# jagannatharjun/AntiZ

Hardware: AMD Instinct MI355X
Metric: input MB/s precompressed (1 GB synthetic, 100k streams) at 1/2/4/8 MI355X (higher is better)
Workload: dtype u8

## Files before the change

antiz_amd/csrc/atz_device.h:

```cpp
#pragma once
#include <stdint.h>

#ifndef ATZ_INF_CLOCKS
#define ATZ_INF_CLOCKS 0
#endif

namespace atz {

struct InfJob {
  uint64_t in_off;
  uint64_t in_len;
  uint64_t out_off;
  uint64_t out_cap;
};
static constexpr uint64_t NO_OUT = ~0ull;
static constexpr uint64_t ARENA_OUT = ~1ull;
static constexpr uint64_t ARENA_NONE = ~0ull;

enum : uint32_t { INF_END = 0, INF_ERROR = 1, INF_NEED = 2, INF_RETRY = 3 };

static constexpr uint32_t INF_HINT_NOSHORT = 1u << 31;
static constexpr uint32_t INF_HINT_MLEV_SHIFT = 27;

struct InfRes {
// ... 81 lines not shown
  TR_FULL = 0,
  TR_SHORTCUT = 1,
  TR_SIZEDIFF = 2,
  TR_CANT_BEAT = 3,
  TR_OVERFLOW = 4,
  TR_NEED_R = 5,
  TR_SKIPPED = 6,
};

struct SweepOpts {
  uint64_t recomp_tresh, sizediff_tresh, shortcut_len, mismatch_tol;
};

__device__ __forceinline__ uint32_t wave_incl_scan(uint32_t v) {
  int x = (int)v;
  x += __builtin_amdgcn_update_dpp(0, x, 0x111, 0xf, 0xf, false);
  x += __builtin_amdgcn_update_dpp(0, x, 0x112, 0xf, 0xf, false);
  x += __builtin_amdgcn_update_dpp(0, x, 0x114, 0xf, 0xf, false);
  x += __builtin_amdgcn_update_dpp(0, x, 0x118, 0xf, 0xf, false);
  x += __builtin_amdgcn_update_dpp(0, x, 0x142, 0xa, 0xf, false);
  x += __builtin_amdgcn_update_dpp(0, x, 0x143, 0xc, 0xf, false);
  return (uint32_t)x;
}

}
```

antiz_amd/csrc/k_deflate.hip:

```cpp
#include <hip/hip_runtime.h>
#include "atz_device.h"

#define LDS __attribute__((address_space(3)))
#define CONSTANT __attribute__((address_space(4)))
#define GLOBAL __attribute__((address_space(1)))

#ifndef ATZ_VISITED_CHECK
#define ATZ_VISITED_CHECK 1
#endif
#ifndef ATZ_VISITED_MAX
#define ATZ_VISITED_MAX 8
#endif
#ifndef ATZ_NOSLIDE_PATH
#define ATZ_NOSLIDE_PATH 1
#endif
#ifndef ATZ_STEP_SPLIT
#define ATZ_STEP_SPLIT 0
#endif
#ifndef ATZ_STEP_CLOCKS
#define ATZ_STEP_CLOCKS 0
#endif
#if ATZ_STEP_CLOCKS
#define STEP_CLOCK() clock64()
#else
// ... 712 lines not shown
  uint32_t heap[HEAPN + 1];
  uint16_t bl_count[16];
  uint32_t blc32[16];
};

struct TreeScratch {
  uint16_t anc[2][HEAPN];
  uint8_t dep[2][HEAPN];
  uint16_t freq[NLC];
};

struct BitOut {
  GLOBAL uint8_t* out;
  uint64_t cap;
  uint64_t pos;
  uint64_t bb;
  uint32_t bc;
  uint32_t raw;
  const GLOBAL uint8_t* orig;
  uint64_t clen;
  uint64_t shortcut;
  uint64_t eq_all;
  uint64_t eq_sc;
  int overflow;
  uint64_t cyc_tree, cyc_emit, blocks;
  uint64_t cyc_heap, cyc_scan, cyc_send;
};

static constexpr uint32_t STAGE_WORDS = 196;
struct BlockFreq {
  uint32_t lfreq2[(NLC + 1) / 2];
  uint32_t dfreq2[NDC / 2];
};
struct TreeCodes {
  uint16_t lcode[NLC]; uint8_t llen[NLC + 2];
  uint16_t dcode[NDC]; uint8_t dlen[NDC + 2];
  uint16_t bcode[NBLC]; uint8_t blen[NBLC + 2];
  uint32_t bfreq[NBLC];
  TreeWork w;
};
struct TrialShared {
  BitOut b;
  BlockFreq f;
  TreeCodes k;
  uint64_t stop_at;
  uint32_t stop_j, pad_;
};

template <uint32_t INS>
struct TrialSharedFast {
  static constexpr uint32_t INS_BITS = INS;
  TrialShared t;
  uint64_t ring[512];
  uint32_t ins[INS / 32];
  uint32_t holes[HOLE_SLOTS];
};

static constexpr uint32_t RING_SLOW = 512;
struct TrialSharedSlow {
  TrialShared t;
  uint64_t ring[RING_SLOW];
};
static_assert(sizeof(TreeScratch) <= RING_SLOW * sizeof(uint64_t), "tree scratch overlays the ring");
static_assert(offsetof(BitOut, cyc_scan) == offsetof(BitOut, cyc_heap) + 8, "block_trees' cyc[0], cyc[1]");
static_assert(STAGE_WORDS * 4 <= RING_SLOW * sizeof(uint64_t), "emission staging overlays the ring");

#ifndef ATZ_MW_F
#define ATZ_MW_F 3
#endif
static constexpr int MW_F = ATZ_MW_F;
struct MWSlot {
  BlockFreq f;
  int64_t block_start;
  uint64_t p, S;
  uint32_t last_lit, sbase, last, seq;
};
struct MWFlusher {
  TreeCodes k;
  TreeScratch sc;
  uint64_t cyc_tree, cyc_emit;
  uint64_t cyc_heap, cyc_scan;
};
static_assert(offsetof(MWFlusher, cyc_scan) == offsetof(MWFlusher, cyc_heap) + 8, "block_trees' cyc[0], cyc[1]");
struct MWCtl {
  uint32_t next_emit;
  uint32_t stop;
  uint32_t parse_done, nblocks;
  uint32_t state, hazard;
// ... 24 lines not shown
__device__ __forceinline__ uint32_t ld_acq(const LDS uint32_t& x) {
  return uni(__hip_atomic_load(&x, __ATOMIC_ACQUIRE, __HIP_MEMORY_SCOPE_WORKGROUP));
}
__device__ __forceinline__ void st_rel(LDS uint32_t& x, uint32_t v, int lane) {
  if (lane == 0) __hip_atomic_store(&x, v, __ATOMIC_RELEASE, __HIP_MEMORY_SCOPE_WORKGROUP);
}

struct SweepArgs {
  const uint8_t* file;
  const uint8_t* infl;
  const uint32_t* chains;
  const uint2* R;
  const StreamDev* streams;
  const Trial* trials;
  TrialRes* res;
  uint32_t* stopj;
  uint8_t* out;
  uint32_t* syms;
  const uint32_t* adler;
  SweepOpts o;
  uint32_t ntrials;
};

__device__ inline uint64_t wsum64(uint64_t v) {
  for (int d = 32; d >= 1; d >>= 1) {
    uint32_t lo = __shfl_xor((uint32_t)v, d, 64), hi = __shfl_xor((uint32_t)(v >> 32), d, 64);
    v += ((uint64_t)hi << 32) | lo;
  }
  return v;
}

__device__ inline void emit_bytes_from_stage(LDS BitOut& b, const LDS uint32_t* stage, uint32_t nb, int lane) {
  uint32_t eqa = 0, eqs = 0;
  nb = uni(nb);
  const uint64_t pos = uni(b.pos), cap = uni(b.cap), clen = uni(b.clen), sc = uni(b.shortcut);
  GLOBAL uint8_t* const out = (GLOBAL uint8_t*)(uintptr_t)uni((uint64_t)(uintptr_t)b.out);
  const GLOBAL uint8_t* const orig = (const GLOBAL uint8_t*)(uintptr_t)uni((uint64_t)(uintptr_t)b.orig);
  for (uint32_t w = (uint32_t)lane; 4 * w < nb; w += 64) {
    const uint32_t word = stage[w];
#pragma unroll
    for (uint32_t j = 0; j < 4; j++) {
      const uint32_t k = 4 * w + j;
      const uint8_t x = (uint8_t)(word >> (8 * j));
      const uint64_t at = pos + k;
      if (k < nb && at < cap) out[at] = x;
      if (k < nb && at < clen) {
        const uint32_t e = orig[at] == x ? 1u : 0u;
        eqa += e;
        if (at < sc) eqs += e;
      }
    }
  }
  b.eq_all += wsum64(eqa);
  b.eq_sc += wsum64(eqs);
  if (pos + nb > cap) b.overflow = 1;
  b.pos = pos + nb;
}

__device__ inline void put_bits(LDS BitOut& b, LDS uint32_t* stage, uint32_t v, uint32_t n, int lane) {
  const uint32_t bc = uni(b.bc) + n;
  const uint64_t bb = uni(b.bb) | ((uint64_t)uni(v) << uni(b.bc));
  if (bc >= 32) {
    if (lane == 0) stage[0] = (uint32_t)bb;
    emit_bytes_from_stage(b, stage, 4, lane);
    b.bb = bb >> 32;
    b.bc = bc - 32;
  } else {
    b.bb = bb;
    b.bc = bc;
  }
}
__device__ inline void flush_bits_bytes(LDS BitOut& b, LDS uint32_t* stage, int lane) {
  const uint32_t bc = uni(b.bc), nb = bc >> 3;
  if (!nb) return;
  const uint64_t bb = uni(b.bb);
  if (lane == 0) { stage[0] = (uint32_t)bb; stage[1] = (uint32_t)(bb >> 32); }
  emit_bytes_from_stage(b, stage, nb, lane);
  b.bb = nb >= 8 ? 0 : (bb >> (8 * nb));
  b.bc = bc - 8 * nb;
}
__device__ inline void windup(LDS BitOut& b, LDS uint32_t* stage, int lane) {
  flush_bits_bytes(b, stage, lane);
  if (uni(b.bc)) {
    if (lane == 0) stage[0] = (uint32_t)b.bb;
    emit_bytes_from_stage(b, stage, 1, lane);
    b.bb = 0; b.bc = 0;
  }
}

__device__ __forceinline__ uint32_t tkey(uint32_t f, uint32_t d, uint32_t n) { return (f << 15) | (d << 10) | n; }

__device__ __forceinline__ void pq_down(LDS uint32_t* heap, int heap_len, int k, int lane) {
  const uint32_t v = uni(heap[k]);
  const uint32_t vk = v >> 10;
  const int t_l = 31 - __builtin_clz((uint32_t)lane + 2u);
  const int off_l = lane + 2 - (1 << t_l);
  for (;;) {
    if (2 * k > heap_len) break;
    const int idx = (k << t_l) + off_l;
    const uint32_t g = (t_l <= 5 && idx <= heap_len) ? heap[idx] : 0xffffffffu;
    int p = k;
    bool stop = false;
    int lj = 0;
#pragma unroll
    for (int t = 1; t <= 5; t++) {
      const uint32_t hl = (uint32_t)__builtin_amdgcn_readlane((int)g, lj);
      const uint32_t hr = (uint32_t)__builtin_amdgcn_readlane((int)g, lj + 1);
      const uint32_t c = (hr >> 10) <= (hl >> 10) ? 1u : 0u;
      const uint32_t hj = c ? hr : hl;
// ... 156 lines not shown
  if (overflow) {
    auto bl = [&](int b) -> uint32_t { return (uint32_t)__builtin_amdgcn_readlane((int)blc, b); };
    auto blset = [&](int b, uint32_t v) { blc = lane == b ? v : blc; };
    do {
      int bits = max_length - 1;
      while (bl(bits) == 0) bits--;
      blset(bits, bl(bits) - 1);
      blset(bits + 1, bl(bits + 1) + 2);
      blset(max_length, bl(max_length) - 1);
      overflow -= 2;
    } while (overflow > 0);
    int h = HEAPN;
    for (int bits = max_length; bits != 0; bits--) {
      uint32_t cnt = bl(bits);
      while (cnt != 0) {
        const uint32_t m = uni(heap[--h]);
        if ((int)m > max_code) continue;
        if (lane == 0) lenv[m] = (uint8_t)bits;
        cnt--;
      }
    }
  }
  if (lane < 16) w.bl_count[lane] = (uint16_t)blc;
  uint64_t o = 0, st = 0;
  for (int n = lane; n < elems && n <= max_code; n += 64) {
    const uint32_t f = sc.freq[n];
    if (f) {
      const uint32_t l = lenv[n];
      const uint32_t xb = (xbits && n >= xbase) ? xbits[n - xbase] : 0u;
      o += (uint64_t)f * (l + xb);
      if (stlen) st += (uint64_t)f * (stlen[n] + xb);
    }
  }
  opt_len += wsum64(o);
  if (stlen) static_len += wsum64(st);
  return TreeRes{max_code, opt_len, static_len};
}

__device__ __noinline__ void gen_codes(const LDS TreeWork& w, int max_code, LDS uint16_t* codes, LDS uint8_t* lens,
                                       int lane) {
  max_code = (int)uni((uint32_t)max_code);
  const bool lb = lane >= 1 && lane <= 15;
  const uint32_t bc = lb ? (uint32_t)w.bl_count[lane] : 0u;
  const uint32_t wv = bc << ((15 - lane) & 15);
  uint32_t nc = lb ? (wave_incl_scan(wv) - wv) >> (15 - lane) : 0u;
  const uint64_t lt = lane ? (~0ull >> (64 - lane)) : 0ull;
  const uint64_t present = __ballot(bc != 0);
  for (int g = 0; g <= max_code; g += 64) {
    const int n = g + lane;
    const uint32_t l = n <= max_code ? lens[n] : 0u;
    uint32_t mine = 0;
    for (uint64_t pm = present; pm; pm &= pm - 1) {
      const int b = __ffsll((unsigned long long)pm) - 1;
      const uint64_t m = __ballot(l == (uint32_t)b);
      if (!m) continue;
      const uint32_t base = (uint32_t)__builtin_amdgcn_readlane((int)nc, b);
      if (l == (uint32_t)b) mine = base + (uint32_t)__popcll(m & lt);
      if (lane == b) nc += (uint32_t)__popcll(m);
// ... 1 lines not shown
    if (n <= max_code && l) codes[n] = (uint16_t)(__builtin_bitreverse32(mine) >> (32 - l));
  }
}

__device__ __forceinline__ uint32_t len_code(uint32_t len) {
  if (len < 8) return len;
  if (len == 255) return 28;
  const uint32_t lg = 31u - (uint32_t)__clz(len);
  return 4u * (lg - 1u) + ((len >> (lg - 2u)) & 3u);
}
__device__ __forceinline__ uint32_t dist_code(uint32_t d) {
  if (d < 4) return d;
  const uint32_t lg = 31u - (uint32_t)__clz(d);
  return 2u * lg + ((d >> (lg - 1u)) & 1u);
}
__device__ __forceinline__ uint32_t lcode_extra(uint32_t c) { return (c < 8 || c == 28) ? 0u : (c - 4) >> 2; }
__device__ __forceinline__ uint32_t lcode_base(uint32_t c) {
  return c < 8 ? c : c == 28 ? 255u : ((4 + (c & 3)) << lcode_extra(c));
}
__device__ __forceinline__ uint32_t dcode_extra(uint32_t d) { return d < 2 ? 0u : (d >> 1) - 1; }
__device__ __forceinline__ uint32_t dcode_base(uint32_t d) { return d < 2 ? d : ((2 + (d & 1)) << dcode_extra(d)); }


__device__ inline uint32_t early_exit(const LDS BitOut& b, const SweepOpts& o, uint64_t best_ident, bool full_needed) {
  if (uni((uint32_t)b.overflow)) return TR_OVERFLOW;
  if (full_needed) return ~0u;
  const uint64_t pos = uni(b.pos), clen = uni(b.clen), sc = uni(b.shortcut);
  if (sc) {
    uint64_t seen = pos < sc ? pos : sc;
    uint64_t mism = seen - uni(b.eq_sc);
    uint64_t thr = o.shortcut_len - o.recomp_tresh;
    if (thr > sc || mism > sc - thr) return TR_SHORTCUT;
  }
  if (pos > clen + o.sizediff_tresh) return TR_SIZEDIFF;
  uint64_t seen = pos < clen ? pos : clen;
  if (clen - (seen - uni(b.eq_all)) <= best_ident) return TR_CANT_BEAT;
  return ~0u;
}

static constexpr uint32_t SYM_PER_LANE = 2;
template <typename C16, typename C8>
__device__ __forceinline__ void sym_bits(uint32_t sy, bool valid, bool end, C16 lc, C8 ll, C16 dc, C8 dl,
                                         uint64_t& v, uint32_t& nb) {
  v = 0; nb = 0;
  if (valid) {
    uint32_t dist = sy >> 8;
    const uint32_t c = sy & 0xff;
    if (dist == 0) {
      v = lc[c]; nb = ll[c];
    } else {
      const uint32_t code = len_code(c);
      v = lc[code + 257]; nb = ll[code + 257];
      const uint32_t xe = lcode_extra(code);
      if (xe) { v |= (uint64_t)(c - lcode_base(code)) << nb; nb += xe; }
      dist--;
      const uint32_t dcd = dist_code(dist);
      v |= (uint64_t)dc[dcd] << nb; nb += dl[dcd];
      const uint32_t xd = dcode_extra(dcd);
      if (xd) { v |= (uint64_t)(dist - dcode_base(dcd)) << nb; nb += xd; }
    }
  } else if (end) {
    v = lc[256]; nb = ll[256];
  }
// ... 67 lines not shown
            if (first) { v64 = cv; nb = cl; }
            v64 |= (uint64_t)s.bcode[16] << nb; nb += s.blen[16];
            v64 |= (uint64_t)(cnt - (first ? 1 : 0) - 3) << nb; nb += 2;
          } else if (cnt <= 10) {
            v64 = s.bcode[17]; nb = s.blen[17];
            v64 |= (uint64_t)(cnt - 3) << nb; nb += 3;
          } else {
            v64 = s.bcode[18]; nb = s.blen[18];
            v64 |= (uint64_t)(cnt - 11) << nb; nb += 7;
          }
        }
      }
    }
    if (send) {
      const uint32_t incl = wave_incl_scan(nb);
      stage_or(stage, off + incl - nb, v64, nb);
      off += (uint32_t)__builtin_amdgcn_readlane((int)incl, 63);
    }
  }
  return off;
}

template <typename C16, typename C8>
__device__ bool compress_block(LDS BitOut& b, LDS uint32_t* stage, const GLOBAL uint32_t* syms, uint32_t nsym,
                               C16 lc, C8 ll, C16 dc, C8 dl, const SweepOpts& o, uint64_t best_ident,
                               bool full_needed, int lane) {
  __builtin_amdgcn_fence(__ATOMIC_ACQ_REL, "workgroup");
  for (uint32_t base = 0; base <= nsym; base += 64 * SYM_PER_LANE) {
    const uint32_t k0 = base + SYM_PER_LANE * (uint32_t)lane;
    const uint64_t sp = *(const GLOBAL uint64_t*)(syms + k0);
    uint64_t v0, v1;
    uint32_t n0, n1;
    sym_bits((uint32_t)sp, k0 < nsym, k0 == nsym, lc, ll, dc, dl, v0, n0);
    sym_bits((uint32_t)(sp >> 32), k0 + 1 < nsym, k0 + 1 == nsym, lc, ll, dc, dl, v1, n1);
    const uint32_t nb = n0 + n1;
    const uint32_t incl = wave_incl_scan(nb);
    const uint32_t total = (uint32_t)__builtin_amdgcn_readlane((int)incl, 63);
    if (total == 0) break;
    for (int i = lane; i < (int)STAGE_WORDS; i += 64) stage[i] = 0;
    const uint32_t bc = uni(b.bc);
    if (lane == 0) { stage[0] = (uint32_t)b.bb; stage[1] = (uint32_t)(b.bb >> 32); }
    const uint32_t off = bc + incl - nb;
    stage_or(stage, off, v0, n0);
    stage_or(stage, off + n0, v1, n1);
    const uint32_t all = bc + total;
    const uint32_t full = all >> 3;
    emit_bytes_from_stage(b, stage, full, lane);
    const uint32_t rem = all & 7;
    const uint32_t lastw = stage[full >> 2];
    b.bb = rem ? ((lastw >> (8 * (full & 3))) & 0xff) & ((1u << rem) - 1) : 0;
    b.bc = rem;
    if (!full_needed && early_exit(b, o, best_ident, false) != ~0u) return true;
  }
  return false;
}

struct Lz {
  uint32_t level, kind, wsize, maxdist, lbs, good, lazy, nice, chain;
  uint32_t n;
  uint32_t p;
  uint32_t lookahead;
  uint32_t S;
  uint32_t block_start;
  uint32_t match_start, prev_match;
  uint32_t match_length, prev_length;
  int match_available;
  uint32_t last_lit;
  uint32_t nsym;
};

// ... 84 lines not shown
                                            int max_blindex, int lane) {
  syms = uni_ptr(syms);
  in = uni_ptr(in);
  block_start = (int64_t)uni((uint64_t)block_start);
  p = uni(p);
  S = uni(S);
  last_lit = uni(last_lit);
  lbs = uni(lbs);
  last = (int)uni((uint32_t)last);
  opt.recomp_tresh = uni(opt.recomp_tresh);
  opt.sizediff_tresh = uni(opt.sizediff_tresh);
  opt.shortcut_len = uni(opt.shortcut_len);
  opt.mismatch_tol = uni(opt.mismatch_tol);
  best_ident = uni(best_ident);
  full_needed = uni((uint32_t)full_needed) != 0;
  opt_lenb = uni(opt_lenb);
  static_lenb = uni(static_lenb);
  lmax = (int)uni((uint32_t)lmax);
  dmax = (int)uni((uint32_t)dmax);
  max_blindex = (int)uni((uint32_t)max_blindex);
  uint32_t hazard = 0;
  const bool bufok = block_start >= (int64_t)S;
  const uint64_t stored_len = (uint64_t)((int64_t)p - block_start);
  const uint64_t blk_start_bytes = b.pos;
  b.blocks++;
  if (stored_len + 4 <= opt_lenb && bufok) {
    put_bits(b, stage, (uint32_t)last, 3, lane);
    windup(b, stage, lane);
    uint32_t len = (uint32_t)stored_len;
    put_bits(b, stage, (len & 0xffff) | ((~len & 0xffff) << 16), 32, lane);
    const GLOBAL uint8_t* src = in + block_start;
    for (uint64_t o = 0; o < stored_len; o += 256) {
      uint32_t nb = stored_len - o < 256 ? (uint32_t)(stored_len - o) : 256u;
      for (uint32_t k = lane; k < 64; k += 64) {
        uint32_t wv = 0;
        for (int q = 0; q < 4; q++) {
          uint32_t at = 4 * k + q;
          if (at < nb) wv |= (uint32_t)src[o + at] << (8 * q);
        }
        stage[k] = wv;
      }
      emit_bytes_from_stage(b, stage, nb, lane);
      if (!full_needed && early_exit(b, opt, best_ident, false) != ~0u) break;
    }
  } else if (static_lenb == opt_lenb) {
    const uint32_t bc0 = uni(b.bc);
    b.bb = uni(b.bb) | ((uint64_t)((1u << 1) + (uint32_t)last) << bc0);
    b.bc = bc0 + 3;
    compress_block(b, stage, syms, last_lit, (const CONSTANT uint16_t*)c_t.st_lcode, (const CONSTANT uint8_t*)c_t.st_llen,
                   (const CONSTANT uint16_t*)c_t.st_dcode, (const CONSTANT uint8_t*)c_t.st_dlen, opt, best_ident,
                   full_needed, lane);
  } else {
    int lcodes = lmax + 1, dcodes = dmax + 1, blcodes = max_blindex + 1;
    const uint64_t cs0 = STEP_CLOCK();
    for (int i = lane; i < (int)STAGE_WORDS; i += 64) stage[i] = 0;
    const uint32_t bc0 = uni(b.bc);
    const uint64_t bb0 = uni(b.bb);
    if (lane == 0) { stage[0] = (uint32_t)bb0; stage[1] = (uint32_t)(bb0 >> 32); }
    uint32_t off = bc0;
    if (lane == 0)
      stage_or(stage, off, (uint64_t)((2u << 1) + (uint32_t)last) | ((uint64_t)(lcodes - 257) << 3) |
                               ((uint64_t)(dcodes - 1) << 8) | ((uint64_t)(blcodes - 4) << 13), 17);
    off += 17;
    if (lane < blcodes) stage_or(stage, off + 3u * (uint32_t)lane, s.blen[bl_order((uint32_t)lane)], 3);
    off += 3u * (uint32_t)blcodes;
    off = rle_tree(s, stage, s.llen, lcodes - 1, true, off, lane);
    off = rle_tree(s, stage, s.dlen, dcodes - 1, true, off, lane);
    {
      const uint32_t full = off >> 3;
      emit_bytes_from_stage(b, stage, full, lane);
      const uint32_t rem = off & 7;
      const uint32_t lastw = stage[full >> 2];
      b.bb = rem ? ((lastw >> (8 * (full & 3))) & 0xff) & ((1u << rem) - 1) : 0;
      b.bc = rem;
    }
    b.cyc_send += STEP_CLOCK() - cs0;
    compress_block(b, stage, syms, last_lit, (const LDS uint16_t*)s.lcode, (const LDS uint8_t*)s.llen,
                   (const LDS uint16_t*)s.dcode, (const LDS uint8_t*)s.dlen, opt, best_ident, full_needed, lane);
  }
  if (b.pos - blk_start_bytes > (uint64_t)lbs + 2ull * last_lit && last_lit) hazard = 1;
  if (last) windup(b, stage, lane);
  return hazard;
}

__device__ __forceinline__ void init_block(LDS BlockFreq& f, int lane) {
  for (int i = lane; i < (NLC + 1) / 2; i += 64) f.lfreq2[i] = 0;
  for (int i = lane; i < NDC / 2; i += 64) f.dfreq2[i] = 0;
  if (lane == 0) f.lfreq2[128] = 1;
}

__device__ __forceinline__ uint32_t flush_block(LDS TrialShared& s, LDS TreeScratch& sc, LDS BitOut& b, const GLOBAL uint32_t* syms,
                                                const GLOBAL uint8_t* in, int64_t block_start, uint64_t p, uint64_t S,
                                                uint32_t last_lit, uint32_t level, uint32_t lbs, int last, const SweepOpts& opt,
                                                uint64_t best_ident, bool full_needed, int lane) {
  const uint64_t c0 = clock64();
  const BlockPlan pl = block_trees(s.f, s.k, sc, &b.cyc_heap, level, (uint64_t)((int64_t)p - block_start), lane);
  const uint64_t c1 = clock64();
  b.cyc_tree += c1 - c0;
  const uint32_t hz = block_emit(s.k, (LDS uint32_t*)&sc, b, syms, in, block_start, p, S, last_lit, lbs, last, opt, best_ident,
                                 full_needed, pl.opt_lenb, pl.static_lenb, pl.lmax, pl.dmax, pl.max_blindex, lane);
  init_block(s.f, lane);
  b.cyc_emit += clock64() - c1;
  return hz;
}
// ... 93 lines not shown
    }
    if (!have) break;
    const int64_t bs = (int64_t)uni((uint64_t)sl.block_start);
    const uint64_t p = uni(sl.p), S = uni(sl.S);
    const uint32_t last_lit = uni(sl.last_lit), sbase = uni(sl.sbase);
    const int last = (int)uni(sl.last);
    const uint64_t c0 = clock64();
    const BlockPlan pl = block_trees(sl.f, me.k, me.sc, &me.cyc_heap, level, (uint64_t)((int64_t)p - bs), lane);
    st_rel(sl.seq, 0u, lane);
    const uint64_t c1 = clock64();
    bool turn = false;
    for (;;) {
      if (ld_acq(ctl.stop)) break;
      if (ld_acq(ctl.next_emit) == k) { turn = true; break; }
      __builtin_amdgcn_s_sleep(1);
    }
    if (!turn) break;
    const uint64_t c2 = clock64();
    const uint32_t hz = uni(block_emit(me.k, stage, b, syms + sbase, in, bs, p, S, last_lit, lbs, last, A.o, tr.best_ident,
                                       full_needed, pl.opt_lenb, pl.static_lenb, pl.lmax, pl.dmax, pl.max_blindex, lane));
    if (hz && lane == 0) __hip_atomic_fetch_or(&ctl.hazard, 1u, __ATOMIC_RELAXED, __HIP_MEMORY_SCOPE_WORKGROUP);
    uint32_t st = ~0u;
    if (last) {
      if (!uni(b.raw)) {
        const uint32_t ad = A.adler[tr.stream];
        const uint32_t be = ((ad >> 24) & 0xff) | ((ad >> 8) & 0xff00) | ((ad << 8) & 0xff0000) | (ad << 24);
        put_bits(b, stage, be, 32, lane);
      }
      flush_bits_bytes(b, stage, lane);
      if (uni((uint32_t)b.overflow)) st = TR_OVERFLOW;
      else if (full_needed) st = TR_FULL;
      else {
        const uint64_t thr = A.o.shortcut_len - A.o.recomp_tresh;
        const uint64_t L = uni(b.pos), clen = uni(b.clen);
        const int64_t dd = (int64_t)(L - clen);
        const uint64_t ad2 = (uint64_t)(dd < 0 ? -dd : dd);
        if (uni(b.shortcut) && uni(b.eq_sc) < thr) st = TR_SHORTCUT;
        else if (ad2 > A.o.sizediff_tresh) st = TR_SIZEDIFF;
        else st = TR_FULL;
      }
    } else {
      st = uni(early_exit(b, A.o, tr.best_ident, full_needed));
    }
    if (lane == 0) { me.cyc_tree += c1 - c0; me.cyc_emit += clock64() - c2; }
    if (last) spec_stop(s, A, tr.best_ident, st, uni(b.eq_all), uni(b.clen), lane);
    if (st != ~0u) {
      if (lane == 0) ctl.state = st;
      st_rel(ctl.stop, 1u, lane);
    }
    st_rel(ctl.next_emit, k + 1, lane);
    if (st != ~0u) break;
  }
}

static constexpr uint32_t TR_DECIDED = 0xfffffffeu;

template <int KIND, typename SH, int STRAT = 0>
struct TrialRun {
  static constexpr bool MW = HasMW<SH>::value;
  static constexpr bool TAB = KIND == 1 || KIND == 2;
  const SweepArgs& A;
  SH& shm;
  const int lane, wave;
  LDS TrialShared& s;
  LDS uint32_t* const stg;
  LDS BitOut& b;
  const uint32_t t;
  const Trial tr;
  const StreamDev sd;
  const uint8_t* const in;
  const uint32_t npad;
  const uint32_t* const sidx;
  const uint32_t* const bpos;
  const bool full_needed;
  const uint64_t lt;
  Lz z;
  bool saving = false, replay = false, rec = false;
  GLOBAL uint32_t* syms = nullptr;
  GLOBAL uint64_t* rtab = nullptr;
  uint32_t sbase = 0;
  uint32_t saved_flags = 0;
  uint32_t run_len = 0, run_imp = 0;
  uint64_t cstart = 0;
  uint32_t rtstart = 0;
  uint32_t hazard = 0;
  uint32_t state = ~0u;
  uint64_t fallbacks = 0, cyc_fb = 0;
  uint64_t csec[4] = {0, 0, 0, 0};
  uint32_t nblk = 0;
  LDS uint64_t* ring = nullptr;
  const GLOBAL uint64_t* Rt = nullptr;
  uint32_t n = 0, wsz = 0, maxd = 0, xlim = 0;
  bool noslide = false;
  uint32_t hi = 0;
  uint64_t pf = 0;
  LDS uint32_t* holes = nullptr;
  LDS uint32_t* ins = nullptr;

  __device__ __forceinline__ TrialRun(const SweepArgs& A_, SH& shm_, int lane_)
      : A(A_), shm(shm_), lane(lane_), wave(MW ? (int)(threadIdx.x >> 6) : 0), s(*(LDS TrialShared*)&shm_.t),
        stg((LDS uint32_t*)shm_.ring), b(s.b), t(blockIdx.x), tr(A_.trials[t]), sd(A_.streams[tr.stream]),
        in(A_.infl + sd.infl_off), npad((uint32_t)((sd.infl_len + 63) & ~63ull)),
        sidx(!TAB ? nullptr : A_.chains + tr.chain_off), bpos(!TAB ? nullptr : sidx + npad),
        full_needed(tr.mode & TM_FULL), lt(lane_ ? (~0ull >> (64 - lane_)) : 0ull) {
    z.level = tr.clevel; z.kind = KIND;
    z.wsize = 1u << tr.window; z.maxdist = z.wsize - LOOKMIN; z.lbs = 1u << (tr.memlevel + 6);
    z.good = c_cfg[z.level][0]; z.lazy = c_cfg[z.level][1]; z.nice = c_cfg[z.level][2]; z.chain = c_cfg[z.level][3];
    z.n = sd.infl_len; z.p = 0; z.lookahead = 0; z.S = 0; z.block_start = 0;
    z.match_start = 0; z.prev_match = 0; z.match_length = 2; z.prev_length = 2; z.match_available = 0;
    z.last_lit = 0; z.nsym = 0;
    if (wave == 0) {
      b.out = (GLOBAL uint8_t*)(A.out + tr.out_off); b.cap = tr.out_cap; b.pos = 0; b.bb = 0; b.bc = 0;
      b.raw = tr.mode & TM_RAW;
      b.orig = (const GLOBAL uint8_t*)(A.file + sd.orig_off); b.clen = sd.comp_len;
      b.shortcut = sd.comp_len > A.o.shortcut_len ? A.o.shortcut_len : 0;
      b.eq_all = 0; b.eq_sc = 0; b.overflow = 0;
    }
    saving = TAB && (tr.mode & TM_SAVE);
    replay = TAB && (tr.mode & TM_REPLAY);
    if (KIND == 2 && replay && (tr.mode & TM_CHECKED)) {
      const uint32_t tlim = tr.x_lim < sd.infl_len ? (uint32_t)tr.x_lim : (uint32_t)sd.infl_len;
      const GLOBAL uint64_t* mt = (const GLOBAL uint64_t*)(A.R + tr.r_off);
      const GLOBAL uint64_t* st = (const GLOBAL uint64_t*)(uintptr_t)tr.rp_tab;
      bool same = true;
      for (uint32_t p0 = 0; p0 < tlim && same; p0 += 256) {
        bool d = false;
#pragma unroll
        for (int u = 0; u < 4; u++) {
          const uint32_t p = p0 + 64u * (uint32_t)u + (uint32_t)lane;
          if (p < tlim) {
            const uint64_t sv = st[p], df = mt[p] ^ sv;
            d |= ((sv & 1ull) && (df & 0xffffff00ull)) || ((sv >> 32) & 1ull && (df & 0xffffff0000000000ull));
          }
        }
        same = __ballot(d) == 0;
      }
      replay = same;
    }
    syms = saving || replay ? (GLOBAL uint32_t*)(uintptr_t)tr.rp_syms : (GLOBAL uint32_t*)(A.syms + tr.sym_off);
    rec = KIND == 2 && saving && (tr.mode & TM_SAVE_TAB);
    rtab = (GLOBAL uint64_t*)(uintptr_t)tr.rp_tab;
    if (rec && wave == 0) {
      for (uint32_t p = (uint32_t)lane; p < sd.infl_len; p += 64) rtab[p] = 0;
      __builtin_amdgcn_fence(__ATOMIC_RELEASE, "workgroup");
    }
    if (wave == 0) {
      b.cyc_tree = b.cyc_emit = b.blocks = 0;
      b.cyc_heap = b.cyc_scan = b.cyc_send = 0;
    }
    cstart = clock64();
    rtstart = (uint32_t)__builtin_amdgcn_s_memrealtime();
    if (wave == 0) init_block(s.f, lane);
    if (wave == 0 && !uni((uint32_t)(tr.mode & TM_RAW))) {
      uint32_t header = (8u + ((uint32_t)(tr.window - 8) << 4)) << 8;
      uint32_t lf = z.level < 2 || KIND >= 3 ? 0 : z.level < 6 ? 1 : z.level == 6 ? 2 : 3;
      header |= lf << 6;
      header += 31 - (header % 31);
      put_bits(b, stg, ((header >> 8) & 0xff) | ((header & 0xff) << 8), 16, lane);
    }
  }

  static constexpr uint32_t ins_mask() { return SH::INS_BITS / 32 - 1; }
  __device__ __forceinline__ bool ins_get(uint32_t q) const { return (ins[(q >> 5) & ins_mask()] >> (q & 31)) & 1u; }
  __device__ __forceinline__ uint32_t S_iter(uint32_t S0, uint32_t q) const {
      uint32_t Sx = S0;
#pragma unroll
      for (int i = 0; i < 2; i++) {
        const bool exh = n <= Sx + 2u * wsz;
        const bool slide = exh ? (q + LOOKMIN > n && q >= Sx + wsz + maxd) : (q > Sx + wsz + maxd);
        if (slide) Sx += wsz;
      }
      return Sx;
  }
  __device__ __forceinline__ bool publish(int last) {
      if constexpr (MW) {
        LDS MWPart& mw = *(LDS MWPart*)&shm.mw;
        const uint32_t f = nblk % (uint32_t)MW_F;
        LDS MWSlot& sl = mw.slot[f];
        for (;;) {
          if (ld_acq(mw.ctl.stop)) return false;
          if (ld_acq(sl.seq) == 0) break;
// ... 53 lines not shown
    if (z.lookahead <= 1) { fill(z); if (z.lookahead == 0) break; }
    z.p += z.lookahead;
    z.lookahead = 0;
    const uint32_t max_start = z.block_start + (uint32_t)max_block;
    if (z.p == 0 || z.p >= max_start) {
      z.lookahead = z.p - max_start;
      z.p = max_start;
      state = FLUSH0();
      if (state != ~0u) break;
    }
    if (z.p - z.block_start >= z.maxdist) {
      state = FLUSH0();
      if (state != ~0u) break;
    }
  }
  }

  __device__ __forceinline__ void parse_replay() {
  const GLOBAL uint32_t* sv = (const GLOBAL uint32_t*)syms;
  const uint32_t nsv = tr.rp_nsym;
  const bool endlit = (tr.rp_flags & 2u) != 0;
  saved_flags |= 4;
  uint32_t k = 0, pos = 0;
  while (k < nsv) {
    const uint32_t cnt = nsv - k < 64u ? nsv - k : 64u;
    const bool valid = (uint32_t)lane < cnt;
    const uint32_t v = valid ? sv[k + (uint32_t)lane] : 0u;
    const uint32_t len = valid ? ((v >> 8) ? (v & 0xffu) + 3u : 1u) : 0u;
    const uint32_t incl = wave_incl_scan(len);
    const uint32_t tot = (uint32_t)__builtin_amdgcn_readlane((int)incl, 63);
    if (xlim < n && pos + tot + 2u > xlim) { state = TR_NEED_R; z.p = pos; break; }
    uint32_t base = 0;
    while (base < cnt) {
      const uint32_t room = z.lbs - 1u - z.last_lit;
      const uint32_t seg_end = cnt - base < room ? cnt : base + room;
      if ((uint32_t)lane >= base && (uint32_t)lane < seg_end) {
        if (v >> 8) {
          const uint32_t lc = 257u + len_code(v & 0xffu), dc = dist_code((v >> 8) - 1u);
          __hip_atomic_fetch_add(&s.f.lfreq2[lc >> 1], 1u << (16 * (lc & 1u)), __ATOMIC_RELAXED, __HIP_MEMORY_SCOPE_WORKGROUP);
          __hip_atomic_fetch_add(&s.f.dfreq2[dc >> 1], 1u << (16 * (dc & 1u)), __ATOMIC_RELAXED, __HIP_MEMORY_SCOPE_WORKGROUP);
        } else {
          __hip_atomic_fetch_add(&s.f.lfreq2[v >> 1], 1u << (16 * (v & 1u)), __ATOMIC_RELAXED, __HIP_MEMORY_SCOPE_WORKGROUP);
        }
      }
      z.last_lit += seg_end - base;
      z.nsym += seg_end - base;
      if (z.last_lit == z.lbs - 1u && !(endlit && k + seg_end == nsv)) {
        z.p = pos + (uint32_t)__builtin_amdgcn_readlane((int)incl, (int)seg_end - 1);
        state = FLUSH0();
        if (state != ~0u) break;
// ... 625 lines not shown
    z.last_lit += cnt;
    z.nsym += cnt;
    q += cnt;
    if (z.last_lit == z.lbs - 1u) {
      z.p = q;
      z.S = S;
      state = FLUSH0();
      if (state != ~0u) break;
    }
  }
  if (state == ~0u) {
    z.p = n;
    z.S = S;
  }
  }

  __device__ __forceinline__ void end_parse() {
  if (MW && state == ~0u) {
    if (publish(1)) saved_flags |= 1;
    else state = TR_DECIDED;
  } else if (state == ~0u) {
    saved_flags |= 1;
    FLUSH(1);
    if (!uni(b.raw)) {
      uint32_t ad = A.adler[tr.stream];
      uint32_t be = ((ad >> 24) & 0xff) | ((ad >> 8) & 0xff00) | ((ad << 8) & 0xff0000) | (ad << 24);
      put_bits(b, stg, be, 32, lane);
    }
    flush_bits_bytes(b, stg, lane);
    if (b.overflow) state = TR_OVERFLOW;
    else if (full_needed) state = TR_FULL;
    else {
      uint64_t thr = A.o.shortcut_len - A.o.recomp_tresh;
      uint64_t L = b.pos;
      int64_t dd = (int64_t)(L - b.clen);
      uint64_t ad2 = (uint64_t)(dd < 0 ? -dd : dd);
      if (b.shortcut && b.eq_sc < thr) state = TR_SHORTCUT;
      else if (ad2 > A.o.sizediff_tresh) state = TR_SIZEDIFF;
      else state = TR_FULL;
    }
    spec_stop(s, A, tr.best_ident, state, uni(b.eq_all), uni(b.clen), lane);
  }
  if constexpr (MW) {
    LDS MWCtl& ctl = (*(LDS MWPart*)&shm.mw).ctl;
    if (lane == 0) ctl.nblocks = nblk;
    st_rel(ctl.parse_done, 1u, lane);
    if (state == TR_NEED_R) st_rel(ctl.stop, 1u, lane);
  }
  }

  __device__ __forceinline__ void finish() {
  if constexpr (MW) {
// ... 146 lines not shown
```

Before: 1726.

## Keep bit-writer state in registers and batch original-byte comparison with prefetch

Moves the deflate bit-output state from LDS into a register struct for the duration of each block. Original-byte comparison now uses aligned word loads with alignbyte and a prefetch of the next chunk. Equality counts are packed into a single 32-bit value and the wave reduction is deferred when a full output is needed. Symbols per lane go from 2 to 4 with a software-prefetched vector load, and small emits use a ballot path instead of LDS staging. In exchange this raises register pressure and adds packed 16-bit counters that rely on static bounds, plus a low-address guard for the word reads.

```diff
diff --git a/antiz_amd/csrc/atz_device.h b/antiz_amd/csrc/atz_device.h
--- a/antiz_amd/csrc/atz_device.h
+++ b/antiz_amd/csrc/atz_device.h
@@ -127,5 +127,8 @@
   x += __builtin_amdgcn_update_dpp(0, x, 0x143, 0xc, 0xf, false);
   return (uint32_t)x;
 }
+__device__ __forceinline__ uint32_t wave_sum(uint32_t v) {
+  return (uint32_t)__builtin_amdgcn_readlane((int)wave_incl_scan(v), 63);
+}
 
 }
diff --git a/antiz_amd/csrc/k_deflate.hip b/antiz_amd/csrc/k_deflate.hip
--- a/antiz_amd/csrc/k_deflate.hip
+++ b/antiz_amd/csrc/k_deflate.hip
@@ -758,12 +758,17 @@
   uint64_t shortcut;
   uint64_t eq_all;
   uint64_t eq_sc;
+  const GLOBAL uint8_t* lo;
   int overflow;
   uint64_t cyc_tree, cyc_emit, blocks;
   uint64_t cyc_heap, cyc_scan, cyc_send;
 };
 
-static constexpr uint32_t STAGE_WORDS = 196;
+#ifndef ATZ_SYM_PER_LANE
+#define ATZ_SYM_PER_LANE 4
+#endif
+static constexpr uint32_t SYM_PER_LANE = ATZ_SYM_PER_LANE;
+static constexpr uint32_t STAGE_WORDS = 64 * SYM_PER_LANE * 48 / 32 + 4;
 struct BlockFreq {
   uint32_t lfreq2[(NLC + 1) / 2];
   uint32_t dfreq2[NDC / 2];
@@ -799,7 +804,9 @@
 };
 static_assert(sizeof(TreeScratch) <= RING_SLOW * sizeof(uint64_t), "tree scratch overlays the ring");
 static_assert(offsetof(BitOut, cyc_scan) == offsetof(BitOut, cyc_heap) + 8, "block_trees' cyc[0], cyc[1]");
-static_assert(STAGE_WORDS * 4 <= RING_SLOW * sizeof(uint64_t), "emission staging overlays the ring");
+static_assert(STAGE_WORDS * 4 <= RING_SLOW * sizeof(uint64_t) && STAGE_WORDS * 4 <= sizeof(TreeScratch),
+              "emission staging overlays the ring (single wave) or the tree scratch (flushers)");
+static_assert(64 * 4 * ((STAGE_WORDS + 63) / 64) < 65536, "emit_bytes_from_stage: packed equal-byte counts");
 
 #ifndef ATZ_MW_F
 #define ATZ_MW_F 3
@@ -870,69 +877,148 @@
   uint32_t ntrials;
 };
 
-__device__ inline uint64_t wsum64(uint64_t v) {
-  for (int d = 32; d >= 1; d >>= 1) {
-    uint32_t lo = __shfl_xor((uint32_t)v, d, 64), hi = __shfl_xor((uint32_t)(v >> 32), d, 64);
-    v += ((uint64_t)hi << 32) | lo;
-  }
-  return v;
-}
-
-__device__ inline void emit_bytes_from_stage(LDS BitOut& b, const LDS uint32_t* stage, uint32_t nb, int lane) {
-  uint32_t eqa = 0, eqs = 0;
+struct BitRegs {
+  GLOBAL uint8_t* out;
+  const GLOBAL uint8_t* orig;
+  uint64_t lo;
+  uint64_t cap, pos, bb, clen, shortcut, eq_all, eq_sc;
+  uint32_t bc, overflow;
+  uint32_t acc;
+  uint64_t pf_pos;
+  uint32_t pf0, pf1;
+};
+__device__ __forceinline__ void orig_prefetch(BitRegs& r, uint64_t pos, int lane);
+__device__ __forceinline__ BitRegs bit_load(const LDS BitOut& b, bool ahead, int lane) {
+  BitRegs r;
+  r.out = (GLOBAL uint8_t*)(uintptr_t)uni((uint64_t)(uintptr_t)b.out);
+  r.orig = (const GLOBAL uint8_t*)(uintptr_t)uni((uint64_t)(uintptr_t)b.orig);
+  r.lo = uni((uint64_t)(uintptr_t)b.lo);
+  r.cap = uni(b.cap); r.pos = uni(b.pos); r.bb = uni(b.bb); r.clen = uni(b.clen); r.shortcut = uni(b.shortcut);
+  r.eq_all = uni(b.eq_all); r.eq_sc = uni(b.eq_sc);
+  r.bc = uni(b.bc); r.overflow = uni((uint32_t)b.overflow);
+  r.acc = 0;
+  r.pf_pos = ~0ull; r.pf0 = r.pf1 = 0;
+  if (ahead) orig_prefetch(r, r.pos, lane);
+  return r;
+}
+__device__ __forceinline__ void bit_store(LDS BitOut& b, BitRegs& r, bool deferred) {
+  if (deferred) {
+    r.eq_all += wave_sum(r.acc & 0xffffu);
+    r.eq_sc += wave_sum(r.acc >> 16);
+    r.acc = 0;
+  }
+  b.pos = r.pos; b.bb = r.bb; b.bc = r.bc;
+  b.eq_all = r.eq_all; b.eq_sc = r.eq_sc;
+  b.overflow = (int)r.overflow;
+}
+
+__device__ __forceinline__ void orig_prefetch(BitRegs& r, uint64_t pos, int lane) {
+  const uint64_t at = pos + 4u * (uint32_t)lane;
+  r.pf_pos = pos;
+  if (at < r.clen) {
+    const uint64_t al = ((uint64_t)(uintptr_t)r.orig + at) & ~3ull;
+    if (al >= r.lo) {
+      const GLOBAL uint32_t* const p = (const GLOBAL uint32_t*)(uintptr_t)al;
+      r.pf0 = p[0]; r.pf1 = p[1];
+    }
+  }
+}
+__device__ __forceinline__ uint32_t orig_word(const BitRegs& r, uint64_t at, uint32_t n, bool pre, uint32_t d0, uint32_t d1) {
+  const uint64_t a = (uint64_t)(uintptr_t)r.orig + at, al = a & ~3ull;
+  if (al >= r.lo) {
+    if (!pre) {
+      const GLOBAL uint32_t* const p = (const GLOBAL uint32_t*)(uintptr_t)al;
+      d0 = p[0]; d1 = p[1];
+    }
+    return __builtin_amdgcn_alignbyte(d1, d0, (uint32_t)a & 3u);
+  }
+  uint32_t w = 0;
+#pragma unroll
+  for (uint32_t j = 0; j < 4; j++)
+    if (j < n) w |= (uint32_t)r.orig[at + j] << (8 * j);
+  return w;
+}
+__device__ inline void emit_bytes_from_stage(BitRegs& r, const LDS uint32_t* stage, uint32_t nb, bool defer, bool ahead,
+                                             int lane) {
   nb = uni(nb);
-  const uint64_t pos = uni(b.pos), cap = uni(b.cap), clen = uni(b.clen), sc = uni(b.shortcut);
-  GLOBAL uint8_t* const out = (GLOBAL uint8_t*)(uintptr_t)uni((uint64_t)(uintptr_t)b.out);
-  const GLOBAL uint8_t* const orig = (const GLOBAL uint8_t*)(uintptr_t)uni((uint64_t)(uintptr_t)b.orig);
-  for (uint32_t w = (uint32_t)lane; 4 * w < nb; w += 64) {
-    const uint32_t word = stage[w];
+  if (!nb) return;
+  const uint64_t pos = r.pos, clen = r.clen, sc = r.shortcut;
+  const bool pre = r.pf_pos == pos;
+  const uint32_t c0 = r.pf0, c1 = r.pf1;
+  if (ahead) orig_prefetch(r, pos + nb, lane);
+  uint32_t eq = 0;
+  for (uint32_t w0 = 0; 4 * w0 < nb; w0 += 64) {
+    const uint32_t w = w0 + (uint32_t)lane, k = 4 * w;
+    if (k < nb) {
+      const uint32_t word = stage[w];
+      const uint32_t nv = nb - k < 4u ? nb - k : 4u;
+      const uint64_t at = pos + k;
+      if (at < clen) {
+        const uint32_t n = clen - at < nv ? (uint32_t)(clen - at) : nv;
+        const uint32_t ns = at >= sc ? 0u : sc - at < n ? (uint32_t)(sc - at) : n;
+        const uint32_t x = word ^ orig_word(r, at, n, pre && w0 == 0, c0, c1);
 #pragma unroll
-    for (uint32_t j = 0; j < 4; j++) {
-      const uint32_t k = 4 * w + j;
-      const uint8_t x = (uint8_t)(word >> (8 * j));
-      const uint64_t at = pos + k;
-      if (k < nb && at < cap) out[at] = x;
-      if (k < nb && at < clen) {
-        const uint32_t e = orig[at] == x ? 1u : 0u;
-        eqa += e;
-        if (at < sc) eqs += e;
-      }
-    }
-  }
-  b.eq_all += wsum64(eqa);
-  b.eq_sc += wsum64(eqs);
-  if (pos + nb > cap) b.overflow = 1;
-  b.pos = pos + nb;
-}
-
-__device__ inline void put_bits(LDS BitOut& b, LDS uint32_t* stage, uint32_t v, uint32_t n, int lane) {
-  const uint32_t bc = uni(b.bc) + n;
-  const uint64_t bb = uni(b.bb) | ((uint64_t)uni(v) << uni(b.bc));
+        for (uint32_t j = 0; j < 4; j++) {
+          const uint32_t e = j < n && ((x >> (8 * j)) & 0xffu) == 0 ? 1u : 0u;
+          eq += e + (j < ns ? e << 16 : 0u);
+        }
+      }
+#pragma unroll
+      for (uint32_t j = 0; j < 4; j++)
+        if (j < nv && at + j < r.cap) r.out[at + j] = (uint8_t)(word >> (8 * j));
+    }
+  }
+  if (defer) r.acc += eq;
+  else {
+    const uint32_t t = wave_sum(eq);
+    r.eq_all += t & 0xffffu;
+    r.eq_sc += t >> 16;
+  }
+  if (pos + nb > r.cap) r.overflow = 1;
+  r.pos = pos + nb;
+}
+__device__ inline void emit_few(BitRegs& r, uint64_t bits, uint32_t n, int lane) {
+  const uint64_t at = r.pos + (uint32_t)lane;
+  bool e = false, es = false;
+  if ((uint32_t)lane < n) {
+    const uint8_t x = (uint8_t)(bits >> (8 * lane));
+    if (at < r.cap) r.out[at] = x;
+    if (at < r.clen) {
+      e = r.orig[at] == x;
+      es = e && at < r.shortcut;
+    }
+  }
+  r.eq_all += (uint32_t)__popcll(__ballot(e));
+  r.eq_sc += (uint32_t)__popcll(__ballot(es));
+  if (r.pos + n > r.cap) r.overflow = 1;
+  r.pos += n;
+}
+
+__device__ inline void put_bits(BitRegs& r, uint32_t v, uint32_t n, int lane) {
+  const uint32_t bc = r.bc + n;
+  const uint64_t bb = r.bb | ((uint64_t)uni(v) << r.bc);
   if (bc >= 32) {
-    if (lane == 0) stage[0] = (uint32_t)bb;
-    emit_bytes_from_stage(b, stage, 4, lane);
-    b.bb = bb >> 32;
-    b.bc = bc - 32;
+    emit_few(r, (uint32_t)bb, 4, lane);
+    r.bb = bb >> 32;
+    r.bc = bc - 32;
   } else {
-    b.bb = bb;
-    b.bc = bc;
-  }
-}
-__device__ inline void flush_bits_bytes(LDS BitOut& b, LDS uint32_t* stage, int lane) {
-  const uint32_t bc = uni(b.bc), nb = bc >> 3;
+    r.bb = bb;
+    r.bc = bc;
+  }
+}
+__device__ inline void flush_bits_bytes(BitRegs& r, int lane) {
+  const uint32_t bc = r.bc, nb = bc >> 3;
   if (!nb) return;
-  const uint64_t bb = uni(b.bb);
-  if (lane == 0) { stage[0] = (uint32_t)bb; stage[1] = (uint32_t)(bb >> 32); }
-  emit_bytes_from_stage(b, stage, nb, lane);
-  b.bb = nb >= 8 ? 0 : (bb >> (8 * nb));
-  b.bc = bc - 8 * nb;
-}
-__device__ inline void windup(LDS BitOut& b, LDS uint32_t* stage, int lane) {
-  flush_bits_bytes(b, stage, lane);
-  if (uni(b.bc)) {
-    if (lane == 0) stage[0] = (uint32_t)b.bb;
-    emit_bytes_from_stage(b, stage, 1, lane);
-    b.bb = 0; b.bc = 0;
+  const uint64_t bb = r.bb;
+  emit_few(r, bb, nb, lane);
+  r.bb = bb >> (8 * nb);
+  r.bc = bc - 8 * nb;
+}
+__device__ inline void windup(BitRegs& r, int lane) {
+  flush_bits_bytes(r, lane);
+  if (r.bc) {
+    emit_few(r, r.bb, 1, lane);
+    r.bb = 0; r.bc = 0;
   }
 }
 
@@ -1135,18 +1221,18 @@
     }
   }
   if (lane < 16) w.bl_count[lane] = (uint16_t)blc;
-  uint64_t o = 0, st = 0;
+  uint32_t o = 0, st = 0;
   for (int n = lane; n < elems && n <= max_code; n += 64) {
     const uint32_t f = sc.freq[n];
     if (f) {
       const uint32_t l = lenv[n];
       const uint32_t xb = (xbits && n >= xbase) ? xbits[n - xbase] : 0u;
-      o += (uint64_t)f * (l + xb);
-      if (stlen) st += (uint64_t)f * (stlen[n] + xb);
-    }
-  }
-  opt_len += wsum64(o);
-  if (stlen) static_len += wsum64(st);
+      o += f * (l + xb);
+      if (stlen) st += f * (stlen[n] + xb);
+    }
+  }
+  opt_len += wave_sum(o);
+  if (stlen) static_len += wave_sum(st);
   return TreeRes{max_code, opt_len, static_len};
 }
 
@@ -1194,7 +1280,8 @@
 __device__ __forceinline__ uint32_t dcode_base(uint32_t d) { return d < 2 ? d : ((2 + (d & 1)) << dcode_extra(d)); }
 
 
-__device__ inline uint32_t early_exit(const LDS BitOut& b, const SweepOpts& o, uint64_t best_ident, bool full_needed) {
+template <typename B>
+__device__ inline uint32_t early_exit(const B& b, const SweepOpts& o, uint64_t best_ident, bool full_needed) {
   if (uni((uint32_t)b.overflow)) return TR_OVERFLOW;
   if (full_needed) return ~0u;
   const uint64_t pos = uni(b.pos), clen = uni(b.clen), sc = uni(b.shortcut);
@@ -1210,7 +1297,6 @@
   return ~0u;
 }
 
-static constexpr uint32_t SYM_PER_LANE = 2;
 template <typename C16, typename C8>
 __device__ __forceinline__ void sym_bits(uint32_t sy, bool valid, bool end, C16 lc, C8 ll, C16 dc, C8 dl,
                                          uint64_t& v, uint32_t& nb) {
@@ -1324,30 +1410,38 @@
 }
 
 template <typename C16, typename C8>
-__device__ bool compress_block(LDS BitOut& b, LDS uint32_t* stage, const GLOBAL uint32_t* syms, uint32_t nsym,
+__device__ bool compress_block(BitRegs& b, LDS uint32_t* stage, const GLOBAL uint32_t* syms, uint32_t nsym,
                                C16 lc, C8 ll, C16 dc, C8 dl, const SweepOpts& o, uint64_t best_ident,
                                bool full_needed, int lane) {
   __builtin_amdgcn_fence(__ATOMIC_ACQ_REL, "workgroup");
+  typedef uint32_t SymVec __attribute__((ext_vector_type(SYM_PER_LANE), aligned(4)));
+  SymVec nx = *(const GLOBAL SymVec*)(syms + SYM_PER_LANE * (uint32_t)lane);
   for (uint32_t base = 0; base <= nsym; base += 64 * SYM_PER_LANE) {
     const uint32_t k0 = base + SYM_PER_LANE * (uint32_t)lane;
-    const uint64_t sp = *(const GLOBAL uint64_t*)(syms + k0);
-    uint64_t v0, v1;
-    uint32_t n0, n1;
-    sym_bits((uint32_t)sp, k0 < nsym, k0 == nsym, lc, ll, dc, dl, v0, n0);
-    sym_bits((uint32_t)(sp >> 32), k0 + 1 < nsym, k0 + 1 == nsym, lc, ll, dc, dl, v1, n1);
-    const uint32_t nb = n0 + n1;
+    const SymVec sp = nx;
+    if (base + 64 * SYM_PER_LANE <= nsym) nx = *(const GLOBAL SymVec*)(syms + k0 + 64 * SYM_PER_LANE);
+    uint64_t v[SYM_PER_LANE];
+    uint32_t n[SYM_PER_LANE], nb = 0;
+#pragma unroll
+    for (uint32_t j = 0; j < SYM_PER_LANE; j++) {
+      sym_bits(sp[j], k0 + j < nsym, k0 + j == nsym, lc, ll, dc, dl, v[j], n[j]);
+      nb += n[j];
+    }
     const uint32_t incl = wave_incl_scan(nb);
     const uint32_t total = (uint32_t)__builtin_amdgcn_readlane((int)incl, 63);
     if (total == 0) break;
-    for (int i = lane; i < (int)STAGE_WORDS; i += 64) stage[i] = 0;
-    const uint32_t bc = uni(b.bc);
+    const uint32_t bc = b.bc;
+    const uint32_t all = bc + total;
+    for (uint32_t i = (uint32_t)lane; i < (all >> 5) + 2 && i < STAGE_WORDS; i += 64) stage[i] = 0;
     if (lane == 0) { stage[0] = (uint32_t)b.bb; stage[1] = (uint32_t)(b.bb >> 32); }
-    const uint32_t off = bc + incl - nb;
-    stage_or(stage, off, v0, n0);
-    stage_or(stage, off + n0, v1, n1);
-    const uint32_t all = bc + total;
+    uint32_t off = bc + incl - nb;
+#pragma unroll
+    for (uint32_t j = 0; j < SYM_PER_LANE; j++) {
+      stage_or(stage, off, v[j], n[j]);
+      off += n[j];
+    }
     const uint32_t full = all >> 3;
-    emit_bytes_from_stage(b, stage, full, lane);
+    emit_bytes_from_stage(b, stage, full, full_needed, true, lane);
     const uint32_t rem = all & 7;
     const uint32_t lastw = stage[full >> 2];
     b.bb = rem ? ((lastw >> (8 * (full & 3))) & 0xff) & ((1u << rem) - 1) : 0;
@@ -1478,13 +1572,15 @@
   uint32_t hazard = 0;
   const bool bufok = block_start >= (int64_t)S;
   const uint64_t stored_len = (uint64_t)((int64_t)p - block_start);
-  const uint64_t blk_start_bytes = b.pos;
   b.blocks++;
+  BitRegs r = bit_load(b, true, lane);
+  const uint64_t blk_start_bytes = r.pos;
   if (stored_len + 4 <= opt_lenb && bufok) {
-    put_bits(b, stage, (uint32_t)last, 3, lane);
-    windup(b, stage, lane);
+    put_bits(r, (uint32_t)last, 3, lane);
+    windup(r, lane);
     uint32_t len = (uint32_t)stored_len;
-    put_bits(b, stage, (len & 0xffff) | ((~len & 0xffff) << 16), 32, lane);
+    put_bits(r, (len & 0xffff) | ((~len & 0xffff) << 16), 32, lane);
+    orig_prefetch(r, r.pos, lane);
     const GLOBAL uint8_t* src = in + block_start;
     for (uint64_t o = 0; o < stored_len; o += 256) {
       uint32_t nb = stored_len - o < 256 ? (uint32_t)(stored_len - o) : 256u;
@@ -1496,22 +1592,21 @@
         }
         stage[k] = wv;
       }
-      emit_bytes_from_stage(b, stage, nb, lane);
-      if (!full_needed && early_exit(b, opt, best_ident, false) != ~0u) break;
+      emit_bytes_from_stage(r, stage, nb, full_needed, true, lane);
+      if (!full_needed && early_exit(r, opt, best_ident, false) != ~0u) break;
     }
   } else if (static_lenb == opt_lenb) {
-    const uint32_t bc0 = uni(b.bc);
-    b.bb = uni(b.bb) | ((uint64_t)((1u << 1) + (uint32_t)last) << bc0);
-    b.bc = bc0 + 3;
-    compress_block(b, stage, syms, last_lit, (const CONSTANT uint16_t*)c_t.st_lcode, (const CONSTANT uint8_t*)c_t.st_llen,
+    r.bb |= (uint64_t)((1u << 1) + (uint32_t)last) << r.bc;
+    r.bc += 3;
+    compress_block(r, stage, syms, last_lit, (const CONSTANT uint16_t*)c_t.st_lcode, (const CONSTANT uint8_t*)c_t.st_llen,
                    (const CONSTANT uint16_t*)c_t.st_dcode, (const CONSTANT uint8_t*)c_t.st_dlen, opt, best_ident,
                    full_needed, lane);
   } else {
     int lcodes = lmax + 1, dcodes = dmax + 1, blcodes = max_blindex + 1;
     const uint64_t cs0 = STEP_CLOCK();
     for (int i = lane; i < (int)STAGE_WORDS; i += 64) stage[i] = 0;
-    const uint32_t bc0 = uni(b.bc);
-    const uint64_t bb0 = uni(b.bb);
+    const uint32_t bc0 = r.bc;
+    const uint64_t bb0 = r.bb;
     if (lane == 0) { stage[0] = (uint32_t)bb0; stage[1] = (uint32_t)(bb0 >> 32); }
     uint32_t off = bc0;
     if (lane == 0)
@@ -1524,18 +1619,19 @@
     off = rle_tree(s, stage, s.dlen, dcodes - 1, true, off, lane);
     {
       const uint32_t full = off >> 3;
-      emit_bytes_from_stage(b, stage, full, lane);
+      emit_bytes_from_stage(r, stage, full, full_needed, true, lane);
       const uint32_t rem = off & 7;
       const uint32_t lastw = stage[full >> 2];
-      b.bb = rem ? ((lastw >> (8 * (full & 3))) & 0xff) & ((1u << rem) - 1) : 0;
-      b.bc = rem;
+      r.bb = rem ? ((lastw >> (8 * (full & 3))) & 0xff) & ((1u << rem) - 1) : 0;
+      r.bc = rem;
     }
     b.cyc_send += STEP_CLOCK() - cs0;
-    compress_block(b, stage, syms, last_lit, (const LDS uint16_t*)s.lcode, (const LDS uint8_t*)s.llen,
+    compress_block(r, stage, syms, last_lit, (const LDS uint16_t*)s.lcode, (const LDS uint8_t*)s.llen,
                    (const LDS uint16_t*)s.dcode, (const LDS uint8_t*)s.dlen, opt, best_ident, full_needed, lane);
   }
-  if (b.pos - blk_start_bytes > (uint64_t)lbs + 2ull * last_lit && last_lit) hazard = 1;
-  if (last) windup(b, stage, lane);
+  if (r.pos - blk_start_bytes > (uint64_t)lbs + 2ull * last_lit && last_lit) hazard = 1;
+  if (last) windup(r, lane);
+  bit_store(b, r, full_needed);
   return hazard;
 }
 
@@ -1675,12 +1771,14 @@
     if (hz && lane == 0) __hip_atomic_fetch_or(&ctl.hazard, 1u, __ATOMIC_RELAXED, __HIP_MEMORY_SCOPE_WORKGROUP);
     uint32_t st = ~0u;
     if (last) {
+      BitRegs r = bit_load(b, false, lane);
       if (!uni(b.raw)) {
         const uint32_t ad = A.adler[tr.stream];
         const uint32_t be = ((ad >> 24) & 0xff) | ((ad >> 8) & 0xff00) | ((ad << 8) & 0xff0000) | (ad << 24);
-        put_bits(b, stage, be, 32, lane);
-      }
-      flush_bits_bytes(b, stage, lane);
+        put_bits(r, be, 32, lane);
+      }
+      flush_bits_bytes(r, lane);
+      bit_store(b, r, false);
       if (uni((uint32_t)b.overflow)) st = TR_OVERFLOW;
       else if (full_needed) st = TR_FULL;
       else {
@@ -1716,7 +1814,6 @@
   SH& shm;
   const int lane, wave;
   LDS TrialShared& s;
-  LDS uint32_t* const stg;
   LDS BitOut& b;
   const uint32_t t;
   const Trial tr;
@@ -1752,7 +1849,7 @@
 
   __device__ __forceinline__ TrialRun(const SweepArgs& A_, SH& shm_, int lane_)
       : A(A_), shm(shm_), lane(lane_), wave(MW ? (int)(threadIdx.x >> 6) : 0), s(*(LDS TrialShared*)&shm_.t),
-        stg((LDS uint32_t*)shm_.ring), b(s.b), t(blockIdx.x), tr(A_.trials[t]), sd(A_.streams[tr.stream]),
+        b(s.b), t(blockIdx.x), tr(A_.trials[t]), sd(A_.streams[tr.stream]),
         in(A_.infl + sd.infl_off), npad((uint32_t)((sd.infl_len + 63) & ~63ull)),
         sidx(!TAB ? nullptr : A_.chains + tr.chain_off), bpos(!TAB ? nullptr : sidx + npad),
         full_needed(tr.mode & TM_FULL), lt(lane_ ? (~0ull >> (64 - lane_)) : 0ull) {
@@ -1766,6 +1863,7 @@
       b.out = (GLOBAL uint8_t*)(A.out + tr.out_off); b.cap = tr.out_cap; b.pos = 0; b.bb = 0; b.bc = 0;
       b.raw = tr.mode & TM_RAW;
       b.orig = (const GLOBAL uint8_t*)(A.file + sd.orig_off); b.clen = sd.comp_len;
+      b.lo = (const GLOBAL uint8_t*)A.file;
       b.shortcut = sd.comp_len > A.o.shortcut_len ? A.o.shortcut_len : 0;
       b.eq_all = 0; b.eq_sc = 0; b.overflow = 0;
     }
@@ -1809,7 +1907,8 @@
       uint32_t lf = z.level < 2 || KIND >= 3 ? 0 : z.level < 6 ? 1 : z.level == 6 ? 2 : 3;
       header |= lf << 6;
       header += 31 - (header % 31);
-      put_bits(b, stg, ((header >> 8) & 0xff) | ((header & 0xff) << 8), 16, lane);
+      b.bb = ((header >> 8) & 0xff) | ((header & 0xff) << 8);
+      b.bc = 16;
     }
   }
 
@@ -1909,10 +2008,13 @@
   const bool endlit = (tr.rp_flags & 2u) != 0;
   saved_flags |= 4;
   uint32_t k = 0, pos = 0;
+  uint32_t nx = (uint32_t)lane < nsv ? sv[lane] : 0u;
   while (k < nsv) {
     const uint32_t cnt = nsv - k < 64u ? nsv - k : 64u;
     const bool valid = (uint32_t)lane < cnt;
-    const uint32_t v = valid ? sv[k + (uint32_t)lane] : 0u;
+    const uint32_t v = nx;
+    if (k + 64u + (uint32_t)lane < nsv) nx = sv[k + 64u + (uint32_t)lane];
+    else nx = 0u;
     const uint32_t len = valid ? ((v >> 8) ? (v & 0xffu) + 3u : 1u) : 0u;
     const uint32_t incl = wave_incl_scan(len);
     const uint32_t tot = (uint32_t)__builtin_amdgcn_readlane((int)incl, 63);
@@ -2584,12 +2686,14 @@
   } else if (state == ~0u) {
     saved_flags |= 1;
     FLUSH(1);
+    BitRegs r = bit_load(b, false, lane);
     if (!uni(b.raw)) {
       uint32_t ad = A.adler[tr.stream];
       uint32_t be = ((ad >> 24) & 0xff) | ((ad >> 8) & 0xff00) | ((ad << 8) & 0xff0000) | (ad << 24);
-      put_bits(b, stg, be, 32, lane);
-    }
-    flush_bits_bytes(b, stg, lane);
+      put_bits(r, be, 32, lane);
+    }
+    flush_bits_bytes(r, lane);
+    bit_store(b, r, false);
     if (b.overflow) state = TR_OVERFLOW;
     else if (full_needed) state = TR_FULL;
     else {
```

New measurement: 1762, median of 6. +2.1%, better.
